# iracigt/ceres-raytracer

Hardware: AMD Instinct MI355X
Metric: Mrays/sec (primary+shadow) on dragon.obj 1920x1080; 1/2/4/8-GPU scaling (higher is better)
Workload: dtype f32; 1 GPU; dragon_1080: dragon.obj 1920x1080 primary+shadow, 16 copies of the config view per step; views=config, W=1920, H=1080, row_block=1080, parallelism=one GPU, whole frames, float_framebuffer=True, streams=8

## Files before the change

ceres-raytracer_amd/__init__.py:

```python
import ctypes
import os
import sys

import numpy as np

_PKG = os.path.dirname(os.path.abspath(__file__))
LIB_PATH = os.environ.get("CERES_LIB") or os.path.join(_PKG, "libceres_hip.so")
CLI_PATH = os.path.join(_PKG, "render")

if _PKG not in sys.path:
    sys.path.insert(0, _PKG)
import configs

MODE_FULL, MODE_PRIMARY = 0, 1
MODE_ROBUST = 0x10
MODE_QBVH4 = 0x20
MODE_FMA = 0x40
ARITH_EXACT, ARITH_FMA = 0, 1


def cfg_mode(cfg, arith=ARITH_EXACT):
    return ((MODE_PRIMARY if cfg["mode"] == "primary" else MODE_FULL) | (MODE_ROBUST if cfg.get("robust") else 0)
            | (MODE_FMA if arith else 0))
SCENE_STATS = 1
SCENE_FIRST_ORDER = 2

EXPORTED_SYMBOLS = (
    "ceres_obj_load", "ceres_proc_mesh", "ceres_rotate_triangles", "ceres_bvh_build", "ceres_bvh_build_gpu",
    "ceres_bvh_build_device", "ceres_obj_load_gpu", "ceres_obj_parse_device", "ceres_rotate_triangles_device",
    "ceres_device_free", "ceres_camera_basis", "ceres_obj_load_f64", "ceres_proc_mesh_f64", "ceres_rotate_triangles_f64",
    "ceres_bvh_build_f64", "ceres_camera_basis_f64", "ceres_orbit_cameras_f64", "ceres_scene_create_f64",
    "ceres_render_f64", "ceres_render_records_f64", "ceres_obj_load_f64_arith", "ceres_proc_mesh_f64_arith",
    "ceres_rotate_triangles_f64_arith", "ceres_bvh_build_f64_arith", "ceres_camera_basis_f64_arith",
    "ceres_orbit_cameras_f64_arith",
    "ceres_free", "ceres_scene_create", "ceres_scene_create_device", "ceres_scene_destroy", "ceres_scene_info", "ceres_scene_shadow_stacks", "ceres_scene_stack_width", "ceres_render_f32",
    "ceres_render_device", "ceres_render_batch_device", "ceres_render_multi_f32", "ceres_device_count", "ceres_assemble_rgb8_packed", "ceres_render_records", "ceres_tiling_local_rows",
    "ceres_scene_set_timing", "ceres_scene_read_timing", "ceres_scene_wave_log", "ceres_fetch_counters",
    "ceres_debug_compact_order", "ceres_debug_kept_tiles",
    "ceres_entry_cut_words", "ceres_entry_cut_build", "ceres_entry_relayout", "ceres_entry_rects", "ceres_entry_tiles",
    "ceres_debug_entry_record", "ceres_debug_entry_nodes",
    "ceres_cpu_scene_create", "ceres_cpu_scene_destroy", "ceres_render_cpu_f32", "ceres_cpu_scene_create_f64",
    "ceres_render_cpu_f64",
    "ceres_orbit_cameras", "ceres_assemble_rgb8",
    "ceres_kernel_names", "ceres_last_error", "ceres_version",
    "ceres_obj_load_arith", "ceres_proc_mesh_arith", "ceres_rotate_triangles_arith", "ceres_bvh_build_arith",
    "ceres_camera_basis_arith", "ceres_orbit_cameras_arith", "ceres_content_hash",
    "ceres_bvh_build_gpu_arith", "ceres_bvh_build_device_arith", "ceres_obj_load_gpu_arith",
    "ceres_obj_parse_device_arith", "ceres_rotate_triangles_device_arith",
    "ceres_trace_rays", "ceres_trace_rays_device", "ceres_trace_rays_cpu",
    "ceres_trace_rays_f64", "ceres_trace_rays_f64_device", "ceres_trace_rays_cpu_f64",
    "ceres_shade_rays", "ceres_shade_rays_device", "ceres_shade_rays_cpu", "ceres_camera_rays",
    "ceres_shade_rays_f64", "ceres_shade_rays_f64_device", "ceres_shade_rays_cpu_f64", "ceres_camera_rays_f64",
    "ceres_scene_refit", "ceres_scene_refit_device", "ceres_scene_refit_f64", "ceres_scene_refit_f64_device",
    "ceres_cpu_scene_refit", "ceres_cpu_scene_refit_f64", "ceres_scene_read_boxes",
    "ceres_scene_sah_cost", "ceres_scene_rebuild", "ceres_scene_rebuild_device", "ceres_scene_update",
# ... 133 lines not shown
    L.ceres_scene_wave_log.argtypes = [_vp, _u64p, _sz, ctypes.POINTER(_sz)]
    L.ceres_fetch_counters.argtypes = [ctypes.c_int, _u64p, ctypes.c_int]
    if hasattr(L, "ceres_debug_compact_order"):
        L.ceres_debug_compact_order.argtypes = [_vp, _u32p, _u32p, _u32p, _sz]
        L.ceres_debug_kept_tiles.argtypes = [_sz, _sz, ctypes.c_uint32, ctypes.c_uint32, ctypes.POINTER(ctypes.c_uint16), _u32p,
                                             _u32p, _sz]
    if hasattr(L, "ceres_entry_cut_build"):
        _u16p = ctypes.POINTER(ctypes.c_uint16)
        L.ceres_entry_cut_words.restype = _sz
        L.ceres_entry_cut_build.argtypes = [_vp, _sz, ctypes.c_uint32, _fp, _u32p]
        L.ceres_entry_relayout.argtypes = [_fp, _sz, _vp, _sz, _u64p, _vp, ctypes.POINTER(_sz), _u32p, _u32p]
        L.ceres_entry_rects.argtypes = [_u32p, _fp, _sz, _sz, _u16p]
        L.ceres_entry_tiles.argtypes = [_u32p, _u16p, _sz, _sz, _u32p]
        L.ceres_debug_entry_record.argtypes = [_vp, ctypes.c_int]
        L.ceres_debug_entry_nodes.argtypes = [_vp, _u32p, _u32p, _u16p, _u32p, _sz]
    L.ceres_cpu_scene_create.argtypes = [_fp, _sz, _fp, _vp, _sz, _u64p]
    L.ceres_cpu_scene_create.restype = _vp
    L.ceres_cpu_scene_destroy.argtypes = [_vp]
    L.ceres_cpu_scene_destroy.restype = None
    L.ceres_render_cpu_f32.argtypes = [_vp, _fp, _fp, ctypes.c_int, _fp, ctypes.POINTER(ctypes.c_uint8), _sz, _sz,
                                       ctypes.POINTER(_Stats), ctypes.c_int]
    L.ceres_cpu_scene_create_f64.argtypes = [_dp, _sz, _dp, _vp, _sz, _u64p]
    L.ceres_cpu_scene_create_f64.restype = _vp
    L.ceres_render_cpu_f64.argtypes = [_vp, _dp, _dp, ctypes.c_int, _dp, ctypes.POINTER(ctypes.c_uint8), _sz, _sz,
                                       ctypes.POINTER(_Stats), ctypes.c_int]
    L.ceres_trace_rays.argtypes = [_vp, _vp, _sz, ctypes.c_int, _vp, _vp, ctypes.POINTER(_Stats)]
    L.ceres_trace_rays_device.argtypes = [_vp, _vp, _sz, ctypes.c_int, _vp, _vp, _vp, _vp]
    L.ceres_trace_rays_cpu.argtypes = [_vp, _vp, _sz, ctypes.c_int, _vp, _vp, ctypes.POINTER(_Stats), ctypes.c_int]
    L.ceres_trace_rays_f64.argtypes = L.ceres_trace_rays.argtypes
    L.ceres_trace_rays_f64_device.argtypes = L.ceres_trace_rays_device.argtypes
# ... 617 lines not shown
    def entry_nodes(self):
        info = np.zeros(8, np.uint32)
        table = np.zeros(cut_words(), np.uint32)
        _check(lib().ceres_debug_entry_nodes(self._h, _p(info, ctypes.c_uint32), _p(table, ctypes.c_uint32), None, None, 0))
        out = {"cut": CutTable(table) if info[0] else None, "used": bool(info[1])}
        if info[1]:
            rects = np.zeros((int(info[2]), 64, 4), np.uint16)
            entries = np.zeros(max(int(info[3]), 1), np.uint32)
            _check(lib().ceres_debug_entry_nodes(self._h, _p(info, ctypes.c_uint32), None, _p(rects, ctypes.c_uint16), None,
                                                 rects.shape[0] * 64))
            _check(lib().ceres_debug_entry_nodes(self._h, _p(info, ctypes.c_uint32), None, None, _p(entries, ctypes.c_uint32),
                                                 len(entries)))
            out.update(rects=rects, entries=entries[:int(info[3])], W=int(info[4]), H=int(info[5]))
        return out

    def read_timing(self):
        p, q, n = ctypes.c_double(), ctypes.c_double(), ctypes.c_uint64()
        _check(lib().ceres_scene_read_timing(self._h, ctypes.byref(p), ctypes.byref(q), ctypes.byref(n)))
        return p.value, q.value, n.value


ENTRY_EMPTY, ENTRY_CULLED = 0xffffffff, 0xfefefefe


def cut_words():
    return int(lib().ceres_entry_cut_words())


class CutTable:

# ... 214 lines not shown
```

ceres-raytracer_amd/csrc/ceres_types.hpp:

```cpp
#pragma once
#include <cstddef>
#include <cstdint>
#include <vector>

namespace ceres {

struct Tri48 {
    float p0[3], e1[3], e2[3], n[3];
};
static_assert(sizeof(Tri48) == 48, "Tri48");

struct RefNode {
    float bounds[6];
    uint32_t primitive_count;
    uint32_t first_child_or_primitive;
};
static_assert(sizeof(RefNode) == 32, "RefNode");

struct alignas(16) SiblingPair {
    float lb[6];
    float rb[6];
    uint32_t lcount, lfirst;
    uint32_t rcount, rfirst;
};
// ... 113 lines not shown
    const QNode4* qnodes4;
    const Tri48* tris;
    const uint32_t* orig;
    const float* norms;
    float* pixels;
    uint8_t* rgb8;
    Shard* shards;
    int32_t* rec_prim;
    float* rec_tuv;
    int8_t* rec_shadow;
    unsigned long long* wave_log;
    uint32_t fill_stride, fill_magic;
    uint32_t n_tiles;
    uint32_t entry_off;
    const uint32_t* cut;
};
constexpr uint32_t kEntryDebug = 0x80000000u;
constexpr uint32_t kEntryEmpty = 0xffffffffu;
constexpr uint32_t kEntryCulled = 0xfefefefeu;

struct CompactArgs {
    uint32_t* buf;
    uint32_t tpw;
    uint32_t deal;
    uint32_t want_tiles;
    uint32_t off_result, off_counts, off_rows;
};
static_assert(sizeof(KParams) + sizeof(CompactArgs) <= 4096, "KParams + CompactArgs must fit the 4 KB kernel-argument limit");
static_assert(sizeof(KParams) <= 4096, "KParams must fit the 4 KB kernel-argument limit");

// ... 27 lines not shown
```

ceres-raytracer_amd/csrc/entry_cut.hpp:

```cpp
#pragma once
#include <cmath>
#include <cstdint>

#include "ceres_types.hpp"

#if defined(__HIPCC__)
#define CERES_CUT_HD __host__ __device__
#else
#define CERES_CUT_HD
#endif

namespace ceres {

constexpr uint32_t kCutMax = 64;
constexpr uint32_t kCutN = 0;
constexpr uint32_t kCutOk = 1;
constexpr uint32_t kCutChecks = 2;
constexpr uint32_t kCutBroken = 3;
constexpr uint32_t kCutSrc = 4;
constexpr uint32_t kCutChild = 68;
constexpr uint32_t kCutBox = 132;
constexpr uint32_t kCutLca = 516;
constexpr uint32_t kCutCheckRec = 4612;
constexpr uint32_t kCutCheckBox = 4740;
// ... 143 lines not shown

CERES_CUT_HD inline bool cut_is_keep(const CullRect& r) { return r.i0 == 0u && r.i1 == 0xffffu && r.j0 == 0u && r.j1 == 0xffffu; }
CERES_CUT_HD inline CullRect cut_lane_rect(const uint32_t* T, const FrameCam& c, uint32_t W, uint32_t H, uint32_t lane) {
    const uint32_t n = T[kCutN];
    if (n < 2u || !T[kCutOk]) return CullRect{0u, 0xffffu, 0u, 0xffffu};
    if (cut_is_keep(box_rect(c, reinterpret_cast<const float*>(T + kCutRootBox), W, H))) return CullRect{0u, 0xffffu, 0u, 0xffffu};
    if (lane >= n) return CullRect{1u, 0u, 1u, 0u};
    return box_rect(c, reinterpret_cast<const float*>(T + kCutBox) + 6 * lane, W, H);
}
CERES_CUT_HD inline bool cut_rect_hits_tile(const CullRect& r, uint32_t W, uint32_t rows, uint32_t bx, uint32_t by) {
    const uint32_t a = 8u * bx, b = a + 7u < W - 1u ? a + 7u : W - 1u;
    const uint32_t p = 8u * by, q = p + 7u < rows - 1u ? p + 7u : rows - 1u;
    return cut_max<uint32_t>(a, r.i0) <= cut_min<uint32_t>(b, r.i1) && cut_max<uint32_t>(p, r.j0) <= cut_min<uint32_t>(q, r.j1);
}

CERES_CUT_HD inline bool cut_words_hit_tile(uint32_t x, uint32_t y, uint32_t W, uint32_t rows, uint32_t bx, uint32_t by) {
    const uint32_t a = 8u * bx, b = a + 7u < W - 1u ? a + 7u : W - 1u;
    const uint32_t p = 8u * by, q = p + 7u < rows - 1u ? p + 7u : rows - 1u;
    return cut_max(a, x & 0xffffu) <= cut_min(b, x >> 16) && cut_max(p, y & 0xffffu) <= cut_min(q, y >> 16);
}

}
```

ceres-raytracer_amd/csrc/render_hip.hip:

```cpp
#include <hip/hip_runtime.h>

#include <algorithm>
#include <chrono>
#include <cfloat>
#include <cmath>
#include <cstdint>
#include <cstdlib>
#include <cstring>
#include <new>
#include <string>
#include <type_traits>
#include <vector>

#include "ceres_render.h"
#include "ceres_types.hpp"
#include "entry_cut.hpp"
#include "host_common.hpp"
#include "pow24.hpp"

#pragma clang fp contract(off)

#ifndef CERES_COUNTING
#define CERES_COUNTING 0
#endif
// ... 51 lines not shown
#ifndef CERES_PK_PACKET
#define CERES_PK_PACKET 1
#endif
#ifndef CERES_LOAD_ALWAYS
#define CERES_LOAD_ALWAYS 1
#endif
#ifndef CERES_CULL
#define CERES_CULL 1
#endif
#ifndef CERES_COMPACT
#define CERES_COMPACT 1
#endif
#ifndef CERES_ENTRY_NODES
#define CERES_ENTRY_NODES 1
#endif
#ifndef CERES_TRI_SELECT
#define CERES_TRI_SELECT 1
#endif

namespace ceres {

char* error_buffer() {
    static thread_local char buf[kErrorBufferSize] = "";
    return buf;
}

namespace dev {

constexpr int kBlock = 256;

// ... 702 lines not shown
    size_t head = mis ? (16u - mis) / sizeof(T) : 0u;
    if (head > n) head = n;
    if (lane < head) p[lane] = T(0);
    p += head; n -= head;
    const size_t nv = n * sizeof(T) / 16;
    uint4* v = reinterpret_cast<uint4*>(p);
    for (size_t k = lane; k < nv; k += 64) v[k] = make_uint4(0u, 0u, 0u, 0u);
    const size_t done = nv * (16 / sizeof(T));
    if (lane < n - done) p[done + lane] = T(0);
}

#ifndef CERES_FILL_SPREAD
#define CERES_FILL_SPREAD 1
#endif

template <bool kBands = false>
__device__ __forceinline__ void fill_culled_rows(const KParams& P, uint32_t task, uint32_t lane) {
    const uint32_t tile_rows = (P.local_rows + 7u) / 8u, tiles_x = (P.W + 7u) / 8u;
    const uint32_t f = task / tile_rows, by = task - f * tile_rows;
    if (f >= P.frames) return;
    const uint32_t lr = by * 8u + (lane & 7u);
    const uint32_t n = __popcll(__ballot(lane < 8u && row_exists<kBands>(P, f, lr)));
    if (!n) return;
    const bool rows_hit = tile_rows_hit<kBands>(P, f, lr);
    uint32_t bx0 = 0, bx1 = 0;
    bool any = false;
    for (uint32_t base = 0; base < tiles_x; base += 64u) {
        const uint64_t m = __ballot(base + lane < tiles_x && !tile_misses_root(P, f, base + lane, rows_hit));
        if (m) {
            if (!any) bx0 = base + uint32_t(__builtin_ctzll(m));
            bx1 = base + 63u - uint32_t(__builtin_clzll(m));
            any = true;
        }
    }
    const size_t W = P.W, frame_base = size_t(f) * P.local_rows;
    if (!any) {
        const size_t lo = by * 8u, hi = lo + n - 1;
        if (P.pixels) zero_run(P.pixels + 3 * ((frame_base + lo) * W), 3 * n * W, lane);
// ... 343 lines not shown
    } else {
        const F3 view = primary_dir<kG>(P, f, i, global_row<kBands>(P, f, lr));
        CERES_COUNT_V(kFShadeV, 40);
        shade<kG>(sun_line, P.norms + 9 * size_t(P.orig[slot]), view, hu, hv, c);
    }
}

constexpr int kFusedB = 64;
constexpr size_t kLdsPerCu = 160 * 1024;
template <bool kStats, typename StkT, int kMinW, bool kRobust, bool kSteal, bool kQ, bool kG, int kTPWo = 0, bool kBands = false,
          bool kEntryDbg = false>
__global__ __launch_bounds__(kFusedB) __attribute__((amdgpu_waves_per_eu(kMinW))) void ceres_fused(const KParams P) {
    constexpr int kB = kFusedB;
    constexpr bool kPacketsCompiled = !kStats && !kSteal && !kRobust && !kQ && CERES_SHADOW_PACKET && std::is_same<StkT, uint16_t*>::value;
    constexpr bool kEntry = CERES_ENTRY_NODES && !kStats && !kSteal && !kRobust && !kQ && !kBands && std::is_same<StkT, uint16_t*>::value;
    extern __shared__ __attribute__((aligned(16))) uint32_t lds[];
    __shared__ StealLdsT<kB> L;
    const uint32_t lane = threadIdx.x, tid = lane;
    constexpr uint32_t kTPWp = (kStats || kSteal) ? 1 : kTPWo ? uint32_t(kTPWo) : uint32_t(CERES_TILES_PER_WAVE);
    constexpr bool kPair = CERES_PAIR_STORES && !kStats && !kSteal && kTPWp >= 2 && std::is_same<StkT, uint16_t*>::value;
    __shared__ typename std::conditional<kPair, PairStash, NoStash>::type S;
    auto tile_pixel = [&](uint32_t t, uint32_t& f_, uint32_t& lr_, uint32_t& i_) {
        uint32_t by_, bx_;
        if (P.tile_packed) {
            bx_ = t & ((1u << kTileXBits) - 1u);
            by_ = (t >> kTileXBits) & ((1u << kTileYBits) - 1u);
            f_ = t >> (kTileXBits + kTileYBits);
        } else {
            const uint32_t per_frame_ = P.tiles_x * P.row_blocks_per_frame;
            f_ = t / per_frame_;
// ... 29 lines not shown
    if constexpr (std::is_same<StkT, Stk24>::value)
        stk = Stk24{reinterpret_cast<uint16_t*>(lds) + tid,
                    reinterpret_cast<uint8_t*>(lds) + size_t(P.lds_entries) * kB * 2 + tid};
    else
        stk = reinterpret_cast<StkT>(lds) + tid;
    constexpr uint32_t kTile = 8;
    constexpr uint32_t kTPW = (kStats || kSteal) ? 1 : kTPWo ? uint32_t(kTPWo) : uint32_t(CERES_TILES_PER_WAVE);
    const uint32_t n_tiles = P.n_tiles;
    uint32_t group = blockIdx.x;
    if constexpr (!kStats) {
        const uint32_t tile_groups = (n_tiles + kTPW - 1) / kTPW;
        if (P.fill_stride) {
            const uint32_t oct = blockIdx.x >> 3, x = blockIdx.x & 7u, nfo = (gridDim.x >> 3) - (tile_groups + 7u) / 8u;
            const uint32_t q = __umulhi(oct, P.fill_magic), r = oct - q * P.fill_stride;
            if (r == P.fill_stride - 1 && q < nfo) {
                fill_culled_rows<kBands>(P, q * 8u + x, lane);
                return;
            }
            group = (oct - (q < nfo ? q : nfo)) * 8u + x;
            if (group >= tile_groups) return;
        } else if (blockIdx.x >= tile_groups) {
            fill_culled_rows<kBands>(P, blockIdx.x - tile_groups, lane);
            return;
        }
    }
    uint32_t n_shadow = 0, occluded = 0, n_pairs = 0, n_tests = 0;
    bool overflow = false;
    static_assert(kTPW == 1 || kTPW == 2 || kTPW == 4 || kTPW == 8, "CERES_TILES_PER_WAVE must be 1, 2, 4 or 8");
    uint4 tiles4 = make_uint4(0, 0, 0, 0), tiles4b = make_uint4(0, 0, 0, 0);
    if constexpr (kTPW == 8) {
        tiles4 = sload_u4(P.tile_order + 8 * size_t(group), 0);
        tiles4b = sload_u4(P.tile_order + 8 * size_t(group), 1);
    } else if constexpr (kTPW == 4) {
        tiles4 = sload_u4(P.tile_order + 4 * size_t(group), 0);
    } else if constexpr (kTPW == 2) {
        tiles4.x = sload_u32(P.tile_order + 2 * size_t(group));
        tiles4.y = sload_u32(P.tile_order + 2 * size_t(group) + 1);
    } else {
        tiles4.x = sload_u32(P.tile_order + group);
    }
    CERES_COUNT_S(kFOrderS, 4 * kTPW);
    const uint32_t n_here = kTPW == 1 || n_tiles - group * kTPW >= kTPW ? kTPW : n_tiles - group * kTPW;
    for (uint32_t q = 0; q < n_here; ++q) {
    const uint4 tq = q < 4 ? tiles4 : tiles4b;
    const uint32_t qq = q & 3;
    const uint32_t t = kTPW == 1 ? tiles4.x : qq == 0 ? tq.x : qq == 1 ? tq.y : qq == 2 ? tq.z : tq.w;
    const uint32_t qp = (q - 1) & 3;
    const uint4 tp = q - 1 < 4 ? tiles4 : tiles4b;
    const uint32_t t_prev = qp == 0 ? tp.x : qp == 1 ? tp.y : qp == 2 ? tp.z : tp.w;
    uint32_t f, lr, i;
    bool active = tile_pixel(t, f, lr, i);
    uint32_t px = (f * P.local_rows + lr) * P.W + i;
    auto redecode = [&]() {
        if constexpr (CERES_LEAN_WRITES) {
// ... 15 lines not shown
    }
    uint32_t entry = 0;
    if constexpr (kEntry) {
        if (P.entry_off) {
            const uint2 r = reinterpret_cast<const uint2*>(P.tile_order + (P.entry_off & ~kEntryDebug))[f * kCutMax + lane];
            const uint64_t reach = __ballot(cut_words_hit_tile(r.x, r.y, P.W, P.local_rows, i >> 3, lr >> 3));
            entry = kEntryEmpty;
            if (reach) {
                const uint32_t lo = uint32_t(__builtin_ctzll(reach)), hi = 63u - uint32_t(__builtin_clzll(reach));
                entry = sload_u32(P.cut + kCutLca + lo * kCutMax + hi);
            }
            if constexpr (kEntryDbg)
                if (lane == 0)
                    const_cast<uint32_t*>(P.tile_order)[(P.entry_off & ~kEntryDebug) + P.frames * 2u * kCutMax +
                                                        (f * P.row_blocks_per_frame + (lr >> 3)) * P.tiles_x + (i >> 3)] = entry;
        }
    }
    if (active && !(kEntry && entry == kEntryEmpty)) {
        const F3 view = primary_dir<kG>(P, f, i, global_row<kBands>(P, f, lr));
        constexpr int kOctMode = (!kSteal || (CERES_OCTANT_SLAB & 4)) ? -1 : -2;
        hit = guarded_trace<kStats, kB, StkT, kRobust, kOctMode, kG>(P, f3(P.cam[f].eye), view, stk, h, n_pairs,
                                                                   n_tests, overflow, entry);
        if (P.rec_prim) {
            redecode();
            P.rec_prim[px] = hit ? int32_t(P.orig[h.slot]) : -1;
            P.rec_tuv[3 * size_t(px)] = hit ? h.t : 0.f;
            P.rec_tuv[3 * size_t(px) + 1] = hit ? h.u : 0.f;
            P.rec_tuv[3 * size_t(px) + 2] = hit ? h.v : 0.f;
            P.rec_shadow[px] = -1;
        }
// ... 65 lines not shown

__global__ __launch_bounds__(256) void ceres_cull_rows(const KParams P, const CompactArgs A) {
    const uint32_t lane = threadIdx.x & 63u, task = blockIdx.x * 4u + (threadIdx.x >> 6);
    const uint32_t tile_rows = P.row_blocks_per_frame;
    const uint32_t f = task / tile_rows, by = task - f * tile_rows;
    if (f >= P.frames) return;
    const bool hit = tile_rows_hit(P, f, by * 8u + (lane & 7u));
    if (lane == 0) A.buf[A.off_rows + task] = hit ? 1u : 0u;
    if (CERES_ENTRY_NODES && P.entry_off && by == 0) {
        const CullRect r = cut_lane_rect(P.cut, P.cam[f], P.W, P.H, lane);
        reinterpret_cast<uint2*>(A.buf + (P.entry_off & ~kEntryDebug))[f * kCutMax + lane] =
            make_uint2(uint32_t(r.i0) | uint32_t(r.i1) << 16, uint32_t(r.j0) | uint32_t(r.j1) << 16);
    }
}

struct Box6 { float b[6]; };
__global__ void ceres_cut_build(const SiblingPair* pairs, uint32_t n_pairs, uint32_t root_leaf_count, Box6 root, uint32_t* T) {
    if (blockIdx.x || threadIdx.x) return;
    cut_build(pairs, n_pairs, root_leaf_count, root.b, T);
}
__global__ __launch_bounds__(128) void ceres_cut_refresh(const SiblingPair* pairs, const float* root_box, uint32_t* T) {
    __shared__ uint32_t bad;
    if (threadIdx.x == 0) bad = 0u;
    __syncthreads();
    if (threadIdx.x < T[kCutN]) cut_load_box(pairs, T, threadIdx.x);
    if (threadIdx.x < 6u) T[kCutRootBox + threadIdx.x] = __float_as_uint(root_box[threadIdx.x]);
    if (threadIdx.x < T[kCutChecks] && !cut_check(pairs, root_box, T, threadIdx.x)) atomicOr(&bad, 1u);
    __syncthreads();
    if (threadIdx.x == 0) T[kCutOk] = (!bad && !T[kCutBroken] && T[kCutN] >= 2u) ? 1u : 0u;
}

__device__ __forceinline__ bool group_kept(const KParams& P, const CompactArgs& A, uint32_t g) {
    bool keep = false;
    for (uint32_t i = 0; i < A.tpw; ++i) {
        const uint32_t p = g * A.tpw + i;
        if (p >= P.n_tiles) break;
        uint32_t f, by, bx;
        order_tile(P, P.tile_order[p], f, by, bx);
        if (f >= P.frames || by >= P.row_blocks_per_frame) continue;
        keep = keep || !tile_misses_root(P, f, bx, A.buf[A.off_rows + f * P.row_blocks_per_frame + by] != 0u);
    }
    return keep;
}

constexpr uint32_t kCompactBlock = 1024;

__device__ __forceinline__ uint32_t block_sum_256(uint32_t x, uint32_t* sh) {
    x = wave_sum(x);
    __syncthreads();
    if ((threadIdx.x & 63u) == 0) sh[threadIdx.x >> 6] = x;
    __syncthreads();
    return sh[0] + sh[1] + sh[2] + sh[3];
}

__global__ __launch_bounds__(256) void ceres_order_count(const KParams P, const CompactArgs A) {
    __shared__ uint32_t sh[4];
    const uint32_t groups = (P.n_tiles + A.tpw - 1u) / A.tpw, g0 = blockIdx.x * kCompactBlock + threadIdx.x * 4u;
    uint32_t c = 0;
    for (uint32_t k = 0; k < 4u; ++k)
        if (g0 + k < groups && group_kept(P, A, g0 + k)) ++c;
    c = block_sum_256(c, sh);
    if (threadIdx.x == 0) A.buf[A.off_counts + blockIdx.x] = c;
}

__global__ __launch_bounds__(256) void ceres_order_compact(const KParams P, const CompactArgs A) {
    __shared__ uint32_t sh[4];
    __shared__ uint32_t wsum[4];
    const uint32_t groups = (P.n_tiles + A.tpw - 1u) / A.tpw, g0 = blockIdx.x * kCompactBlock + threadIdx.x * 4u;
    uint32_t before = 0, total = 0;
    for (uint32_t b = threadIdx.x; b < gridDim.x; b += 256u) {
        const uint32_t c = A.buf[A.off_counts + b];
        total += c;
// ... 16 lines not shown
    for (uint32_t off = 1; off < 64u; off <<= 1) {
        const uint32_t y = __shfl_up(x, off, 64);
        if (lane >= off) x += y;
    }
    if (lane == 63u) wsum[wave] = x;
    __syncthreads();
    uint32_t k = before + x - mine;
    for (uint32_t w = 0; w < wave; ++w) k += wsum[w];
    for (uint32_t j = 0; j < 4u; ++j) {
        if (!keep[j]) continue;
        uint32_t slot = k++;
        if (slot < dealt) {
            const uint32_t r = slot % run;
            slot = slot - r + (r % A.deal) * 8u + r / A.deal;
        }
        for (uint32_t i = 0; i < A.tpw; ++i) {
            const uint32_t p = (g0 + j) * A.tpw + i;
            A.buf[slot * A.tpw + i] = p < P.n_tiles ? P.tile_order[p] : 0u;
        }
    }
    if (blockIdx.x == gridDim.x - 1u) {
        const uint32_t end = total * A.tpw, padded = (kept_tiles + 7u) / 8u * 8u;
        if (end + threadIdx.x < padded) A.buf[end + threadIdx.x] = 0u;
        if (threadIdx.x == 0) {
            A.buf[A.off_result] = total;
            A.buf[A.off_result + 1] = kept_tiles;
            if (kept_tiles != A.want_tiles) atomicOr(&P.shards[0].error, 2u);
        }
    }
}

__global__ __launch_bounds__(256) void ceres_compact_lit(const float* __restrict__ px, uint32_t n_pix,
                                                         uint4* __restrict__ out, uint32_t* __restrict__ n,
                                                         uint32_t cap) {
// ... 824 lines not shown
            P.row_blocks_per_frame = fby;
            uint32_t n_tiles = fbx * fby * frames;
            bool compacted = false;
            if (CERES_COMPACT && P.cull && fill_tasks && tile_order->d_curve && tpw > 1 && P.packets) {
                const uint32_t kept = count_kept_tiles(P, *tile_order, tpw);
                if (kept < n_tiles) {
                    const uint32_t groups = (n_tiles + tpw - 1) / tpw, nb = (groups + dev::kCompactBlock - 1) / dev::kCompactBlock;
                    ceres::CompactArgs A{};
                    A.tpw = tpw; A.deal = tile_order->deal; A.want_tiles = kept;
                    A.off_result = (groups * tpw + 8u + 3u) / 4u * 4u;
                    A.off_counts = A.off_result + 4u;
                    A.off_rows = A.off_counts + nb;
                    const bool entry = CERES_ENTRY_NODES && s->d_cut && !robust && !qbvh && st16;
                    const uint32_t off_entry = (A.off_rows + frames * fby + 1u) / 2u * 2u;
                    const size_t entry_words = !entry ? 0 : size_t(frames) * 2u * kCutMax + (s->entry_debug ? size_t(n_tiles) : 0);
                    ceres_scene::CompactBuf* cb = nullptr;
                    if (int rc = compact_buffer(s, stream, size_t(off_entry) + entry_words, &cb)) return rc;
                    if (entry) {
                        P.entry_off = off_entry | (s->entry_debug ? kEntryDebug : 0u);
                        P.cut = s->d_cut;
                    }
                    cb->entry_off = P.entry_off; cb->frames = frames; cb->W = P.W; cb->H = P.H;
                    if (P.entry_off & kEntryDebug)
                        HIP_TRY(hipMemsetAsync(cb->d + off_entry + size_t(frames) * 2u * kCutMax, 0xfe, size_t(n_tiles) * sizeof(uint32_t), stream));
                    A.buf = cb->d;
                    KParams Q = P;
                    Q.tile_order = tile_order->d_curve;
                    Q.n_tiles = n_tiles;
                    hipLaunchKernelGGL(dev::ceres_cull_rows, dim3((frames * fby + 3u) / 4u), dim3(256), 0, stream, Q, A);
                    hipLaunchKernelGGL(dev::ceres_order_count, dim3(nb), dim3(256), 0, stream, Q, A);
                    hipLaunchKernelGGL(dev::ceres_order_compact, dim3(nb), dim3(256), 0, stream, Q, A);
                    HIP_TRY(hipGetLastError());
                    cb->src = tile_order->d_curve; cb->n = n_tiles; cb->host_tiles = kept; cb->tpw = tpw;
                    cb->deal = A.deal; cb->off_result = A.off_result;
                    P.tile_order = cb->d;
                    n_tiles = kept;
                    compacted = true;
                }
            }
            if (!stats && frames > 1) { s->last_fused_stream = stream; s->last_fused_compacted = compacted; }
            P.n_tiles = n_tiles;
            const uint32_t tile_groups = (n_tiles + tpw - 1) / tpw;
            dim3 fgrid(tile_groups + fill_tasks), fblock(dev::kFusedB);
            if (CERES_FILL_SPREAD > (steal ? 1 : 0) && fill_tasks) {
                const uint64_t nto = (tile_groups + 7) / 8, nfo = (fill_tasks + 7) / 8, stride = (nto + nfo) / nfo;
// ... 1073 lines not shown
        if (cap < n_rect) return set_error(CERES_EINVAL, "ceres_debug_entry_nodes: %u rectangles needed", n_rect);
        std::vector<uint32_t> w(size_t(n_rect) * 2);
        HIP_TRY(hipMemcpy(w.data(), b->d + off, w.size() * sizeof(uint32_t), hipMemcpyDeviceToHost));
        for (size_t k = 0; k < n_rect; ++k) {
            rects[4 * k] = uint16_t(w[2 * k]); rects[4 * k + 1] = uint16_t(w[2 * k] >> 16);
            rects[4 * k + 2] = uint16_t(w[2 * k + 1]); rects[4 * k + 3] = uint16_t(w[2 * k + 1] >> 16);
        }
    }
    if (entries && n_entries) {
        if (cap < n_entries) return set_error(CERES_EINVAL, "ceres_debug_entry_nodes: %u entries needed", n_entries);
        HIP_TRY(hipMemcpy(entries, b->d + off + size_t(n_rect) * 2, size_t(n_entries) * sizeof(uint32_t), hipMemcpyDeviceToHost));
    }
    return CERES_OK;
}

int ceres_fetch_counters(int device, uint64_t out[8], int reset) {
    if (!out) return set_error(CERES_EINVAL, "ceres_fetch_counters: null argument");
#if CERES_COUNTING
    static_assert(dev::kFKinds == 8, "ceres_fetch_counters reports 8 kinds");
    HIP_TRY(hipSetDevice(device));
    HIP_TRY(hipDeviceSynchronize());
    unsigned long long h[dev::kFetchShards][dev::kFKinds];
    HIP_TRY(hipMemcpyFromSymbol(h, HIP_SYMBOL(dev::g_fetch), sizeof h));
    for (int k = 0; k < dev::kFKinds; ++k) {
        out[k] = 0;
        for (int q = 0; q < dev::kFetchShards; ++q) out[k] += h[q][k];
    }
    if (reset) {
        std::memset(h, 0, sizeof h);
        HIP_TRY(hipMemcpyToSymbol(HIP_SYMBOL(dev::g_fetch), h, sizeof h));
// ... 37 lines not shown
```

ceres-raytracer_amd/csrc/scene_internal.hpp:

```cpp
#pragma once
#include <hip/hip_runtime.h>

#include <cstdint>
#include <utility>
#include <vector>

#include "ceres_types.hpp"

using ceres::SiblingPair; using ceres::SiblingPair64; using ceres::Node4; using ceres::Tri48; using ceres::Tri96;
using ceres::Shard;

struct ceres_scene {
    int device = 0;
    uint32_t flags = 0;
    size_t n_tri = 0, n_pairs = 0;
    uint32_t depth = 0, stack_entries = 1, root_leaf_count = 0, root_leaf_first = 0;
    float root_box[6] = {0, 0, 0, 0, 0, 0};
    uint32_t root_box_ok = 0;
    uint32_t shadow_stack_entries = 1;
    uint32_t shadow_stack_first = 1;
    size_t n_nodes4 = 0;
    int debug_stack_width = 0;
    SiblingPair* d_pairs = nullptr;
    Node4* d_nodes4 = nullptr;
// ... 11 lines not shown
            uint32_t w = 0, h = 0;
            std::vector<int32_t> sum;
        };
        std::vector<SubsetBoxes> shapes;
        std::vector<uint32_t> h_curve;
        bool countable = false;
    };
    struct CompactBuf {
        hipStream_t stream = nullptr;
        uint32_t* d = nullptr;
        size_t cap = 0;
        uint64_t used = 0;
        const uint32_t* src = nullptr;
        uint32_t n = 0, host_tiles = 0, tpw = 0, deal = 0, off_result = 0;
        uint32_t entry_off = 0, frames = 0, W = 0, H = 0;
    };
    uint32_t* d_cut = nullptr;
    bool entry_debug = false;
    std::vector<CompactBuf> compact;
    hipStream_t last_fused_stream = nullptr;
    bool last_fused_compacted = false;
    std::vector<TileOrder> orders;
    std::vector<uint32_t*> retired;
    size_t retired_bytes = 0;
    uint64_t order_clock = 0;
    Tri48* d_tris = nullptr;
    uint32_t* d_orig = nullptr;
    float* d_norms = nullptr;
    Shard* d_shards = nullptr;
    bool shards_dirty = true;
// ... 61 lines not shown
```

include/ceres_render.h:

```cpp
#ifndef CERES_RENDER_H
#define CERES_RENDER_H

#include <stddef.h>
#include <stdint.h>

#ifdef __cplusplus
extern "C" {
#endif

typedef enum {
    CERES_OK = 0,
    CERES_EINVAL = -1,
    CERES_EIO = -2,
    CERES_ENOMEM = -3,
    CERES_EHIP = -4,
    CERES_ESTACK = -5,
    CERES_EUNSUPPORTED = -6
} ceres_status;

typedef enum {
    CERES_MODE_FULL = 0,
    CERES_MODE_PRIMARY = 1,
    CERES_MODE_ROBUST = 0x10,
    CERES_MODE_QBVH4 = 0x20,
// ... 178 lines not shown

int ceres_scene_wave_log(ceres_scene* scene, uint64_t* out, size_t max_waves, size_t* n_waves);

int ceres_debug_compact_order(ceres_scene* scene, uint32_t info[8], uint32_t* order, uint32_t* source, size_t cap);
int ceres_debug_kept_tiles(size_t width, size_t height, uint32_t frames, uint32_t tiles_per_wave, const uint16_t* rects,
                           uint32_t info[4], uint32_t* source, size_t cap);

size_t ceres_entry_cut_words(void);
int ceres_entry_cut_build(const void* pairs64, size_t n_pairs, uint32_t root_leaf_count, const float root_box[6], uint32_t* table);
int ceres_entry_relayout(const float* tri48, size_t n_tri, const void* nodes32, size_t n_nodes, const uint64_t* prim64,
                         void* pairs64, size_t* n_pairs, uint32_t* orig, uint32_t* root_leaf_count);
int ceres_entry_rects(const uint32_t* table, const float basis12[12], size_t width, size_t height, uint16_t* rects);
int ceres_entry_tiles(const uint32_t* table, const uint16_t* rects, size_t width, size_t height, uint32_t* entries);
int ceres_debug_entry_record(ceres_scene* scene, int enable);
int ceres_debug_entry_nodes(ceres_scene* scene, uint32_t info[8], uint32_t* table, uint16_t* rects, uint32_t* entries, size_t cap);

int ceres_fetch_counters(int device, uint64_t out[8], int reset);

typedef struct ceres_cpu_scene ceres_cpu_scene;
ceres_cpu_scene* ceres_cpu_scene_create(const float* tri48, size_t n_tri, const float* norm36, const void* nodes32,
                                        size_t n_nodes, const uint64_t* prim64);
void ceres_cpu_scene_destroy(ceres_cpu_scene* scene);
int ceres_render_cpu_f32(const ceres_cpu_scene* scene, const float basis12[12], const float sun[3], int mode,
                         float* pixels, uint8_t* rgb8, size_t width, size_t height, ceres_stats* stats, int threads);
ceres_cpu_scene* ceres_cpu_scene_create_f64(const double* tri96, size_t n_tri, const double* norm72, const void* nodes64,
                                            size_t n_nodes, const uint64_t* prim64);
int ceres_render_cpu_f64(const ceres_cpu_scene* scene, const double basis12[12], const double sun[3], int mode,
                         double* pixels, uint8_t* rgb8, size_t width, size_t height, ceres_stats* stats, int threads);
int ceres_cpu_scene_refit(ceres_cpu_scene* scene, const float* tri48, size_t n_tri, const float* norm36);
int ceres_cpu_scene_refit_f64(ceres_cpu_scene* scene, const double* tri96, size_t n_tri, const double* norm72);
// ... 30 lines not shown
```

Before: 54150 Mrays/s.

## Retire tiles whose entry cut is empty before the fused trace kernel

During compaction, an extra set of blocks in the order-count kernel builds a per-row bitmask of tiles that overlap some entry-cut rectangle. The compact kernel uses it to write a per-group flag, so fused-kernel waves whose tiles are all dead exit right after loading their tile indices. The fill path zeroes every non-live run of a row from the mask, and per-tile empty entries skip tracing. This aims to cut wasted traversal and launch work on background pixels, at the cost of a larger compaction buffer, extra mask-building work and a new debug readback API.

```diff
diff --git a/ceres-raytracer_amd/__init__.py b/ceres-raytracer_amd/__init__.py
--- a/ceres-raytracer_amd/__init__.py
+++ b/ceres-raytracer_amd/__init__.py
@@ -38,7 +38,7 @@
     "ceres_scene_set_timing", "ceres_scene_read_timing", "ceres_scene_wave_log", "ceres_fetch_counters",
     "ceres_debug_compact_order", "ceres_debug_kept_tiles",
     "ceres_entry_cut_words", "ceres_entry_cut_build", "ceres_entry_relayout", "ceres_entry_rects", "ceres_entry_tiles",
-    "ceres_debug_entry_record", "ceres_debug_entry_nodes",
+    "ceres_debug_entry_record", "ceres_debug_entry_nodes", "ceres_debug_retire",
     "ceres_cpu_scene_create", "ceres_cpu_scene_destroy", "ceres_render_cpu_f32", "ceres_cpu_scene_create_f64",
     "ceres_render_cpu_f64",
     "ceres_orbit_cameras", "ceres_assemble_rgb8",
@@ -202,6 +202,8 @@
         L.ceres_entry_tiles.argtypes = [_u32p, _u16p, _sz, _sz, _u32p]
         L.ceres_debug_entry_record.argtypes = [_vp, ctypes.c_int]
         L.ceres_debug_entry_nodes.argtypes = [_vp, _u32p, _u32p, _u16p, _u32p, _sz]
+    if hasattr(L, "ceres_debug_retire"):
+        L.ceres_debug_retire.argtypes = [_vp, _u32p, _u32p, ctypes.POINTER(ctypes.c_uint8), _sz]
     L.ceres_cpu_scene_create.argtypes = [_fp, _sz, _fp, _vp, _sz, _u64p]
     L.ceres_cpu_scene_create.restype = _vp
     L.ceres_cpu_scene_destroy.argtypes = [_vp]
@@ -849,6 +851,21 @@
             out.update(rects=rects, entries=entries[:int(info[3])], W=int(info[4]), H=int(info[5]))
         return out
 
+    def retire(self):
+        info = np.zeros(8, np.uint32)
+        _check(lib().ceres_debug_retire(self._h, _p(info, ctypes.c_uint32), None, None, 0))
+        if not info[0]:
+            return None
+        frames, rows, mw, W = int(info[1]), int(info[2]), int(info[3]), int(info[6])
+        mask = np.zeros(max(int(info[4]), 1), np.uint32)
+        flags = np.zeros(max(int(info[5]), 1), np.uint8)
+        _check(lib().ceres_debug_retire(self._h, _p(info, ctypes.c_uint32), _p(mask, ctypes.c_uint32), None, len(mask)))
+        _check(lib().ceres_debug_retire(self._h, _p(info, ctypes.c_uint32), None, _p(flags, ctypes.c_uint8), len(flags)))
+        words = mask[:frames * rows * mw].reshape(frames, rows, mw)
+        bits = (words[..., None] >> np.arange(32, dtype=np.uint32)) & 1
+        live = bits.reshape(frames, rows, mw * 32)[:, :, :(W + 7) // 8].astype(bool)
+        return {"live": live, "words": words, "flags": flags[:int(info[5])], "W": W, "H": int(info[7])}
+
     def read_timing(self):
         p, q, n = ctypes.c_double(), ctypes.c_double(), ctypes.c_uint64()
         _check(lib().ceres_scene_read_timing(self._h, ctypes.byref(p), ctypes.byref(q), ctypes.byref(n)))
diff --git a/ceres-raytracer_amd/csrc/ceres_types.hpp b/ceres-raytracer_amd/csrc/ceres_types.hpp
--- a/ceres-raytracer_amd/csrc/ceres_types.hpp
+++ b/ceres-raytracer_amd/csrc/ceres_types.hpp
@@ -151,6 +151,7 @@
     uint32_t n_tiles;
     uint32_t entry_off;
     const uint32_t* cut;
+    uint32_t retire_off, flag_off;
 };
 constexpr uint32_t kEntryDebug = 0x80000000u;
 constexpr uint32_t kEntryEmpty = 0xffffffffu;
diff --git a/ceres-raytracer_amd/csrc/entry_cut.hpp b/ceres-raytracer_amd/csrc/entry_cut.hpp
--- a/ceres-raytracer_amd/csrc/entry_cut.hpp
+++ b/ceres-raytracer_amd/csrc/entry_cut.hpp
@@ -181,10 +181,13 @@
     return cut_max<uint32_t>(a, r.i0) <= cut_min<uint32_t>(b, r.i1) && cut_max<uint32_t>(p, r.j0) <= cut_min<uint32_t>(q, r.j1);
 }
 
+CERES_CUT_HD inline bool cut_words_hit_rows(uint32_t y, uint32_t rows, uint32_t by) {
+    const uint32_t p = 8u * by, q = p + 7u < rows - 1u ? p + 7u : rows - 1u;
+    return cut_max(p, y & 0xffffu) <= cut_min(q, y >> 16);
+}
 CERES_CUT_HD inline bool cut_words_hit_tile(uint32_t x, uint32_t y, uint32_t W, uint32_t rows, uint32_t bx, uint32_t by) {
     const uint32_t a = 8u * bx, b = a + 7u < W - 1u ? a + 7u : W - 1u;
-    const uint32_t p = 8u * by, q = p + 7u < rows - 1u ? p + 7u : rows - 1u;
-    return cut_max(a, x & 0xffffu) <= cut_min(b, x >> 16) && cut_max(p, y & 0xffffu) <= cut_min(q, y >> 16);
+    return cut_max(a, x & 0xffffu) <= cut_min(b, x >> 16) && cut_words_hit_rows(y, rows, by);
 }
 
 }
diff --git a/ceres-raytracer_amd/csrc/render_hip.hip b/ceres-raytracer_amd/csrc/render_hip.hip
--- a/ceres-raytracer_amd/csrc/render_hip.hip
+++ b/ceres-raytracer_amd/csrc/render_hip.hip
@@ -89,6 +89,12 @@
 #ifndef CERES_ENTRY_NODES
 #define CERES_ENTRY_NODES 1
 #endif
+#ifndef CERES_RETIRE_EMPTY
+#define CERES_RETIRE_EMPTY 1
+#endif
+#ifndef CERES_RETIRE_EXIT
+#define CERES_RETIRE_EXIT 1
+#endif
 #ifndef CERES_TRI_SELECT
 #define CERES_TRI_SELECT 1
 #endif
@@ -821,7 +827,44 @@
 #define CERES_FILL_SPREAD 1
 #endif
 
-template <bool kBands = false>
+__device__ __forceinline__ void fill_retired_runs(const KParams& P, uint32_t f, uint32_t by, uint32_t n, uint32_t lane) {
+    const uint32_t tile_rows = (P.local_rows + 7u) / 8u, tiles_x = (P.W + 7u) / 8u, mw = (tiles_x + 31u) / 32u;
+    const uint32_t* mask = P.tile_order + P.retire_off + size_t(f * tile_rows + by) * mw;
+    const size_t W = P.W, frame_base = size_t(f) * P.local_rows;
+    uint32_t any = 0;
+    for (uint32_t w = 0; w < mw; ++w) any |= sload_u32(mask + w);
+    if (!any) {
+        const size_t lo = by * 8u, hi = lo + n - 1;
+        if (P.pixels) zero_run(P.pixels + 3 * ((frame_base + lo) * W), 3 * n * W, lane);
+        if (P.rgb8) zero_run(P.rgb8 + 3 * ((frame_base + (P.local_rows - 1 - hi)) * W), 3 * n * W, lane);
+        return;
+    }
+    auto run = [&](uint32_t bx0, uint32_t bx1) {
+        const size_t a = size_t(bx0) * 8u, b = size_t(bx1) * 8u < W ? size_t(bx1) * 8u : W;
+        for (uint32_t k = 0; k < n; ++k) {
+            const size_t row = by * 8u + k;
+            if (P.pixels) zero_run(P.pixels + 3 * ((frame_base + row) * W + a), 3 * (b - a), lane);
+            if (P.rgb8) zero_run(P.rgb8 + 3 * ((frame_base + (P.local_rows - 1 - row)) * W + a), 3 * (b - a), lane);
+        }
+    };
+    uint32_t start = 0;
+    bool open = false;
+    for (uint32_t w = 0; w < mw; ++w) {
+        const uint32_t base = w * 32u, nb = tiles_x - base < 32u ? tiles_x - base : 32u, m = sload_u32(mask + w);
+        for (uint32_t pos = 0; pos < nb;) {
+            const uint32_t rest = (open ? m : ~m) >> pos;
+            if (!rest) break;
+            pos += uint32_t(__builtin_ctz(rest));
+            if (pos >= nb) break;
+            if (open) run(start, base + pos);
+            else start = base + pos;
+            open = !open;
+        }
+    }
+    if (open) run(start, tiles_x);
+}
+
+template <bool kBands = false, bool kRetire = false>
 __device__ __forceinline__ void fill_culled_rows(const KParams& P, uint32_t task, uint32_t lane) {
     const uint32_t tile_rows = (P.local_rows + 7u) / 8u, tiles_x = (P.W + 7u) / 8u;
     const uint32_t f = task / tile_rows, by = task - f * tile_rows;
@@ -829,6 +872,11 @@
     const uint32_t lr = by * 8u + (lane & 7u);
     const uint32_t n = __popcll(__ballot(lane < 8u && row_exists<kBands>(P, f, lr)));
     if (!n) return;
+    if constexpr (kRetire && !kBands)
+        if (P.retire_off) {
+            fill_retired_runs(P, f, by, n, lane);
+            return;
+        }
     const bool rows_hit = tile_rows_hit<kBands>(P, f, lr);
     uint32_t bx0 = 0, bx1 = 0;
     bool any = false;
@@ -1202,6 +1250,7 @@
     constexpr int kB = kFusedB;
     constexpr bool kPacketsCompiled = !kStats && !kSteal && !kRobust && !kQ && CERES_SHADOW_PACKET && std::is_same<StkT, uint16_t*>::value;
     constexpr bool kEntry = CERES_ENTRY_NODES && !kStats && !kSteal && !kRobust && !kQ && !kBands && std::is_same<StkT, uint16_t*>::value;
+    constexpr bool kRetire = kEntry && CERES_RETIRE_EMPTY;
     extern __shared__ __attribute__((aligned(16))) uint32_t lds[];
     __shared__ StealLdsT<kB> L;
     const uint32_t lane = threadIdx.x, tid = lane;
@@ -1261,19 +1310,22 @@
             const uint32_t oct = blockIdx.x >> 3, x = blockIdx.x & 7u, nfo = (gridDim.x >> 3) - (tile_groups + 7u) / 8u;
             const uint32_t q = __umulhi(oct, P.fill_magic), r = oct - q * P.fill_stride;
             if (r == P.fill_stride - 1 && q < nfo) {
-                fill_culled_rows<kBands>(P, q * 8u + x, lane);
+                fill_culled_rows<kBands, kRetire>(P, q * 8u + x, lane);
                 return;
             }
             group = (oct - (q < nfo ? q : nfo)) * 8u + x;
             if (group >= tile_groups) return;
         } else if (blockIdx.x >= tile_groups) {
-            fill_culled_rows<kBands>(P, blockIdx.x - tile_groups, lane);
+            fill_culled_rows<kBands, kRetire>(P, blockIdx.x - tile_groups, lane);
             return;
         }
     }
     uint32_t n_shadow = 0, occluded = 0, n_pairs = 0, n_tests = 0;
     bool overflow = false;
     static_assert(kTPW == 1 || kTPW == 2 || kTPW == 4 || kTPW == 8, "CERES_TILES_PER_WAVE must be 1, 2, 4 or 8");
+    uint32_t retire_flags = 0;
+    if constexpr (kRetire && !kEntryDbg && CERES_RETIRE_EXIT)
+        if (P.flag_off) retire_flags = sload_u32(P.tile_order + P.flag_off + (group >> 2));
     uint4 tiles4 = make_uint4(0, 0, 0, 0), tiles4b = make_uint4(0, 0, 0, 0);
     if constexpr (kTPW == 8) {
         tiles4 = sload_u4(P.tile_order + 8 * size_t(group), 0);
@@ -1285,6 +1337,9 @@
         tiles4.y = sload_u32(P.tile_order + 2 * size_t(group) + 1);
     } else {
         tiles4.x = sload_u32(P.tile_order + group);
+    }
+    if constexpr (kRetire && !kEntryDbg && CERES_RETIRE_EXIT) {
+        if (retire_flags && ((retire_flags >> ((group & 3u) * 8u)) & 0xffu)) return;
     }
     CERES_COUNT_S(kFOrderS, 4 * kTPW);
     const uint32_t n_here = kTPW == 1 || n_tiles - group * kTPW >= kTPW ? kTPW : n_tiles - group * kTPW;
@@ -1330,6 +1385,11 @@
                 if (lane == 0)
                     const_cast<uint32_t*>(P.tile_order)[(P.entry_off & ~kEntryDebug) + P.frames * 2u * kCutMax +
                                                         (f * P.row_blocks_per_frame + (lr >> 3)) * P.tiles_x + (i >> 3)] = entry;
+            if constexpr (kRetire)
+                if (entry == kEntryEmpty) {
+                    if (stashed) flush(t_prev);
+                    continue;
+                }
         }
     }
     if (active && !(kEntry && entry == kEntryEmpty)) {
@@ -1425,6 +1485,30 @@
     }
 }
 
+__device__ __forceinline__ void live_mask_chunk(const KParams& P, const CompactArgs& A, uint32_t task, uint32_t lane) {
+    const uint32_t tile_rows = P.row_blocks_per_frame, chunks = (P.tiles_x + 63u) / 64u;
+    const uint32_t row = task / chunks, base = (task - row * chunks) * 64u;
+    const uint32_t f = row / tile_rows, by = row - f * tile_rows;
+    if (f >= P.frames) return;
+    const uint32_t bx = base + lane;
+    const bool rows_hit = A.buf[A.off_rows + row] != 0u;
+    bool live = false;
+    if (__ballot(bx < P.tiles_x && !tile_misses_root(P, f, bx, rows_hit))) {
+        const uint2 r = reinterpret_cast<const uint2*>(A.buf + (P.entry_off & ~kEntryDebug))[f * kCutMax + lane];
+        for (uint64_t c = __ballot(cut_words_hit_rows(r.y, P.local_rows, by)); c; c &= c - 1u) {
+            const int k = __builtin_ctzll(c);
+            const uint32_t xk = uint32_t(__builtin_amdgcn_readlane(int(r.x), k)), yk = uint32_t(__builtin_amdgcn_readlane(int(r.y), k));
+            live = live || cut_words_hit_tile(xk, yk, P.W, P.local_rows, bx, by);
+        }
+    }
+    const uint64_t m = __ballot(bx < P.tiles_x && live && !tile_misses_root(P, f, bx, rows_hit));
+    if (lane == 0) {
+        uint32_t* mask = A.buf + P.retire_off + size_t(row) * ((P.tiles_x + 31u) / 32u);
+        mask[base >> 5] = uint32_t(m);
+        if (base + 32u < P.tiles_x) mask[(base >> 5) + 1u] = uint32_t(m >> 32);
+    }
+}
+
 struct Box6 { float b[6]; };
 __global__ void ceres_cut_build(const SiblingPair* pairs, uint32_t n_pairs, uint32_t root_leaf_count, Box6 root, uint32_t* T) {
     if (blockIdx.x || threadIdx.x) return;
@@ -1454,6 +1538,13 @@
     return keep;
 }
 
+__device__ __forceinline__ bool tile_live(const KParams& P, const CompactArgs& A, uint32_t t) {
+    uint32_t f, by, bx;
+    order_tile(P, t, f, by, bx);
+    if (f >= P.frames || by >= P.row_blocks_per_frame || bx >= P.tiles_x) return false;
+    return (A.buf[P.retire_off + size_t(f * P.row_blocks_per_frame + by) * ((P.tiles_x + 31u) / 32u) + (bx >> 5)] >> (bx & 31u)) & 1u;
+}
+
 constexpr uint32_t kCompactBlock = 1024;
 
 __device__ __forceinline__ uint32_t block_sum_256(uint32_t x, uint32_t* sh) {
@@ -1467,6 +1558,11 @@
 __global__ __launch_bounds__(256) void ceres_order_count(const KParams P, const CompactArgs A) {
     __shared__ uint32_t sh[4];
     const uint32_t groups = (P.n_tiles + A.tpw - 1u) / A.tpw, g0 = blockIdx.x * kCompactBlock + threadIdx.x * 4u;
+    const uint32_t count_blocks = (groups + kCompactBlock - 1u) / kCompactBlock;
+    if (CERES_RETIRE_EMPTY && blockIdx.x >= count_blocks) {
+        if (P.retire_off) live_mask_chunk(P, A, (blockIdx.x - count_blocks) * 4u + (threadIdx.x >> 6), threadIdx.x & 63u);
+        return;
+    }
     uint32_t c = 0;
     for (uint32_t k = 0; k < 4u; ++k)
         if (g0 + k < groups && group_kept(P, A, g0 + k)) ++c;
@@ -1513,10 +1609,13 @@
             const uint32_t r = slot % run;
             slot = slot - r + (r % A.deal) * 8u + r / A.deal;
         }
+        bool live = false;
         for (uint32_t i = 0; i < A.tpw; ++i) {
-            const uint32_t p = (g0 + j) * A.tpw + i;
-            A.buf[slot * A.tpw + i] = p < P.n_tiles ? P.tile_order[p] : 0u;
-        }
+            const uint32_t p = (g0 + j) * A.tpw + i, t = p < P.n_tiles ? P.tile_order[p] : 0u;
+            A.buf[slot * A.tpw + i] = t;
+            if (CERES_RETIRE_EMPTY && P.flag_off && p < P.n_tiles) live = tile_live(P, A, t) || live;
+        }
+        if (CERES_RETIRE_EMPTY && P.flag_off) reinterpret_cast<uint8_t*>(A.buf + P.flag_off)[slot] = live ? 0u : 1u;
     }
     if (blockIdx.x == gridDim.x - 1u) {
         const uint32_t end = total * A.tpw, padded = (kept_tiles + 7u) / 8u * 8u;
@@ -2371,13 +2470,20 @@
                     const bool entry = CERES_ENTRY_NODES && s->d_cut && !robust && !qbvh && st16;
                     const uint32_t off_entry = (A.off_rows + frames * fby + 1u) / 2u * 2u;
                     const size_t entry_words = !entry ? 0 : size_t(frames) * 2u * kCutMax + (s->entry_debug ? size_t(n_tiles) : 0);
+                    const bool retire = CERES_RETIRE_EMPTY && entry;
+                    const size_t mask_words = !retire ? 0 : size_t(frames) * fby * ((fbx + 31u) / 32u);
+                    const size_t off_mask = size_t(off_entry) + entry_words, off_flags = off_mask + mask_words;
+                    const size_t flag_words = !retire ? 0 : (size_t(groups) + 3u) / 4u;
+                    if (off_flags + flag_words > 0x7fffffffu) return set_error(CERES_EINVAL, "render: the batch's compaction buffer exceeds 2^31 words");
                     ceres_scene::CompactBuf* cb = nullptr;
-                    if (int rc = compact_buffer(s, stream, size_t(off_entry) + entry_words, &cb)) return rc;
+                    if (int rc = compact_buffer(s, stream, off_flags + flag_words, &cb)) return rc;
                     if (entry) {
                         P.entry_off = off_entry | (s->entry_debug ? kEntryDebug : 0u);
                         P.cut = s->d_cut;
                     }
+                    if (retire) { P.retire_off = uint32_t(off_mask); P.flag_off = uint32_t(off_flags); }
                     cb->entry_off = P.entry_off; cb->frames = frames; cb->W = P.W; cb->H = P.H;
+                    cb->retire_off = P.retire_off; cb->flag_off = P.flag_off;
                     if (P.entry_off & kEntryDebug)
                         HIP_TRY(hipMemsetAsync(cb->d + off_entry + size_t(frames) * 2u * kCutMax, 0xfe, size_t(n_tiles) * sizeof(uint32_t), stream));
                     A.buf = cb->d;
@@ -2385,7 +2491,7 @@
                     Q.tile_order = tile_order->d_curve;
                     Q.n_tiles = n_tiles;
                     hipLaunchKernelGGL(dev::ceres_cull_rows, dim3((frames * fby + 3u) / 4u), dim3(256), 0, stream, Q, A);
-                    hipLaunchKernelGGL(dev::ceres_order_count, dim3(nb), dim3(256), 0, stream, Q, A);
+                    hipLaunchKernelGGL(dev::ceres_order_count, dim3(nb + (retire ? (frames * fby * ((fbx + 63u) / 64u) + 3u) / 4u : 0u)), dim3(256), 0, stream, Q, A);
                     hipLaunchKernelGGL(dev::ceres_order_compact, dim3(nb), dim3(256), 0, stream, Q, A);
                     HIP_TRY(hipGetLastError());
                     cb->src = tile_order->d_curve; cb->n = n_tiles; cb->host_tiles = kept; cb->tpw = tpw;
@@ -3489,6 +3595,35 @@
     return CERES_OK;
 }
 
+int ceres_debug_retire(ceres_scene* s, uint32_t info[8], uint32_t* mask, uint8_t* flags, size_t cap) {
+    if (!s || !info) return set_error(CERES_EINVAL, "ceres_debug_retire: null argument");
+    for (int k = 0; k < 8; ++k) info[k] = 0;
+    if (!s->last_fused_compacted) return CERES_OK;
+    const ceres_scene::CompactBuf* b = nullptr;
+    for (const auto& c : s->compact)
+        if (c.stream == s->last_fused_stream) b = &c;
+    if (!b || !b->d) return set_error(CERES_EINVAL, "ceres_debug_retire: the launch's buffer is gone");
+    if (!b->retire_off) return CERES_OK;
+    HIP_TRY(hipSetDevice(s->device));
+    HIP_TRY(hipStreamSynchronize(b->stream));
+    uint32_t res[2] = {0, 0};
+    HIP_TRY(hipMemcpy(res, b->d + b->off_result, sizeof res, hipMemcpyDeviceToHost));
+    const uint32_t tile_rows = (b->H + 7u) / 8u, mw = ((b->W + 7u) / 8u + 31u) / 32u;
+    const size_t mask_words = size_t(b->frames) * tile_rows * mw;
+    const size_t n_flags = std::min<size_t>(res[0], (size_t(b->n) + b->tpw - 1) / b->tpw);
+    info[0] = 1; info[1] = b->frames; info[2] = tile_rows; info[3] = mw; info[4] = uint32_t(mask_words); info[5] = uint32_t(n_flags);
+    info[6] = b->W; info[7] = b->H;
+    if (mask) {
+        if (cap < mask_words) return set_error(CERES_EINVAL, "ceres_debug_retire: %zu mask words needed", mask_words);
+        HIP_TRY(hipMemcpy(mask, b->d + b->retire_off, mask_words * sizeof(uint32_t), hipMemcpyDeviceToHost));
+    }
+    if (flags && n_flags) {
+        if (cap < n_flags) return set_error(CERES_EINVAL, "ceres_debug_retire: %zu flags needed", n_flags);
+        HIP_TRY(hipMemcpy(flags, b->d + b->flag_off, n_flags, hipMemcpyDeviceToHost));
+    }
+    return CERES_OK;
+}
+
 int ceres_fetch_counters(int device, uint64_t out[8], int reset) {
     if (!out) return set_error(CERES_EINVAL, "ceres_fetch_counters: null argument");
 #if CERES_COUNTING
diff --git a/ceres-raytracer_amd/csrc/scene_internal.hpp b/ceres-raytracer_amd/csrc/scene_internal.hpp
--- a/ceres-raytracer_amd/csrc/scene_internal.hpp
+++ b/ceres-raytracer_amd/csrc/scene_internal.hpp
@@ -49,6 +49,7 @@
         const uint32_t* src = nullptr;
         uint32_t n = 0, host_tiles = 0, tpw = 0, deal = 0, off_result = 0;
         uint32_t entry_off = 0, frames = 0, W = 0, H = 0;
+        uint32_t retire_off = 0, flag_off = 0;
     };
     uint32_t* d_cut = nullptr;
     bool entry_debug = false;
diff --git a/include/ceres_render.h b/include/ceres_render.h
--- a/include/ceres_render.h
+++ b/include/ceres_render.h
@@ -216,6 +216,7 @@
 int ceres_entry_tiles(const uint32_t* table, const uint16_t* rects, size_t width, size_t height, uint32_t* entries);
 int ceres_debug_entry_record(ceres_scene* scene, int enable);
 int ceres_debug_entry_nodes(ceres_scene* scene, uint32_t info[8], uint32_t* table, uint16_t* rects, uint32_t* entries, size_t cap);
+int ceres_debug_retire(ceres_scene* scene, uint32_t info[8], uint32_t* mask, uint8_t* flags, size_t cap);
 
 int ceres_fetch_counters(int device, uint64_t out[8], int reset);
 
```

New measurement: 55220 Mrays/s, median of 6. 2.0% higher.
